# RhushabhVaghela/Custom-NVComp-with-ZSTD

Hardware: AMD Instinct MI355X
Metric: compress GB/s + ratio, 1 GB @ level 3, 64 KB chunks; libzstd round-trip OK (higher is better)
Workload: dtype u8; 1 GPU; C3: 16384 x 64 KiB chunks (1.00 GiB), level 3, independent frames; chunk_bytes=65536, chunks_total=16384, chunks_rank0=16384, level=3, parallelism=dp1 (contiguous chunk shards, RCCL all-gather of sizes inside the step), gathered_frame_bytes=388747049

## Files before the change

custom-nvcomp-with-zstd_amd/csrc/zh_lz.hip:

```cpp
#include "zh_common.h"
#include "zh_hash.h"
#include "zh_litpack.h"

#include <algorithm>
#include <vector>

#if defined(ZH_STAMPS) || defined(ZH_INS_CHECK)
__device__ u32 g_fixups;
extern "C" __global__ void zh_read_fixups(u32 *out) { *out = g_fixups; g_fixups = 0; }
extern "C" u32 zh_fixups_host() {
  u32 *d = nullptr, h = 0;
  if (hipMalloc(&d, 4) != hipSuccess) return ~0u;
  hipLaunchKernelGGL(zh_read_fixups, dim3(1), dim3(1), 0, 0, d);
  (void)hipMemcpy(&h, d, 4, hipMemcpyDeviceToHost);
  (void)hipFree(d);
  return h;
}
#endif
#ifdef ZH_TIMELINE
__device__ unsigned long long g_tl[16 * 8];
extern "C" __global__ void zh_read_timeline(unsigned long long *out) {
  for (u32 i = threadIdx.x; i < 16 * 8; i += blockDim.x) { out[i] = g_tl[i]; g_tl[i] = 0; }
}
extern "C" int zh_timeline_host(unsigned long long *out128) {
// ... 293 lines not shown
__device__ __forceinline__ u32 lookahead(const u32 *in32, const u16 *T, u32 we, u32 lim, u32 lane) {
  u32 cwe = 0;
  if (lane < 2 && we + lane < lim) {
    u32 lo, hi;
    ld64u(in32, we + lane, lo, hi);
    cwe = T[hash_of<LONG>(lo, hi)];
  }
  __asm__ volatile("" ::: "memory");
  return cwe;
}
struct NoCheck {
  __device__ bool operator()(bool) const { return true; }
};

template <bool LONG>
__device__ __forceinline__ void insert_span(const u32 *in32, u16 *T, u32 s, u32 e, u32 lane) {
  constexpr u32 JUNK = LONG ? HL_SIZE : HS_SIZE;
  for (u32 r = s; r < e; r += 64) {
    u32 const p = r + lane;
    bool const v = p < e;
    u32 lo, hi;
    ld64u(in32, v ? p : s, lo, hi);
    u32 const h = v ? hash_of<LONG>(lo, hi) : JUNK;
    T[h] = (u16)(p + 1);
    for (;;) {
      bool const lost = v && (u32)T[h] < p + 1;
      if (!__ballot(lost)) break;
      if (lost) T[h] = (u16)(p + 1);
    }
  }
  __asm__ volatile("" ::: "memory");
}

__device__ __forceinline__ bool skip_window(const u32 *misc, u32 k, u32 kskip0) {
  return k >= kskip0 && (u32)__builtin_amdgcn_readfirstlane(__atomic_load_n(&misc[MISC_NM + ((k - 3) & 3)], __ATOMIC_RELAXED)) == 0;
}
__device__ __forceinline__ bool skip_window_eff(const u32 *misc, u32 k, u32 kskip0) {
#ifdef ZH_NO_RESUME
  return skip_window(misc, k, kskip0);
#endif
  return skip_window(misc, k, kskip0) && (u32)__builtin_amdgcn_readfirstlane(__atomic_load_n(&misc[MISC_RESF + (k & 1)], __ATOMIC_RELAXED)) == 0;
}
template <bool LONG, bool TWO>
__device__ __forceinline__ bool resume_exchange(u32 *misc, u32 j, bool hit, u32 lane) {
  if constexpr (TWO) {
    u32 *const x = &misc[MISC_XCH + 2 * (j & 1)];
    if (lane == 0) __atomic_store_n(&x[LONG ? 1 : 0], ((j + 1) << 1) | (hit ? 1u : 0u), __ATOMIC_RELAXED);
    u32 v;
    for (;;) {
      v = (u32)__builtin_amdgcn_readfirstlane(__atomic_load_n(&x[LONG ? 0 : 1], __ATOMIC_RELAXED));
      if ((v >> 1) == j + 1) break;
      __builtin_amdgcn_s_sleep(1);
    }
    hit = hit || (v & 1u);
  }
  if (lane == 0) __atomic_store_n(&misc[MISC_RESF + (j & 1)], hit ? 1u : 0u, __ATOMIC_RELAXED);
  return hit;
}

__device__ __forceinline__ bool probe_dead(const u32 *misc, u32 k, u32 kprobe) {
  if (ZH_PROBE_WINDOWS == 1 || k != kprobe) return false;
  u32 m = 0;
#pragma unroll
  for (u32 j = 1; j <= ZH_PROBE_WINDOWS; j++) m |= __atomic_load_n(&misc[MISC_NM + ((k - 1 - j) & 3)], __ATOMIC_RELAXED);
  return (u32)__builtin_amdgcn_readfirstlane(m) == 0;
}
static_assert(ZH_PROBE_WINDOWS >= 1 && ZH_PROBE_WINDOWS <= 3, "probe windows fit the match-count ring");
constexpr u32 span_top_mask(u64 tab) {
  u32 m = 0, hi = 0;
  for (u32 w = 1; w + 1 < INS_TID / 64; w++) {
    hi += (u32)((tab >> (2 * w)) & 3u);
    m |= 1u << hi;
  }
  return m;
}
__device__ __forceinline__ bool span_top_dec(const u32 *ci, u32 wn, bool skip, u32 L, bool act) {
  constexpr u32 TOPS_FULL = span_top_mask(ROUND_TAB), TOPS_SKIP = ((1u << (2 * ZH_SKIP_TILES)) - 1u) & ~1u;
  u32 const hi = L + 1, i = 64 * hi - 1;
  bool const top = act && L < NROUND && (((skip ? TOPS_SKIP : TOPS_FULL) >> hi) & 1u) && i < wn;
  u32 const inf = top ? ci[cidx(i)] : 0u, inf1 = top ? ci[cidx(i + 1)] : 0u;
  return top && (inf & 255u) && (inf1 & 255u) <= (inf & 255u);
}
__device__ __forceinline__ bool probe_dead_tm(u32 k, u32 kprobe, u32 e0, bool lazy = false, u32 wnp = 0) {
  if (ZH_PROBE_WINDOWS != 1 || k + 1 != kprobe) return false;
  u8 *const smem = k1_lds();
  u32 lane;
  __asm__ volatile("v_mbcnt_lo_u32_b32 %0, -1, 0\n\tv_mbcnt_hi_u32_b32 %0, -1, %0" : "=v"(lane));
  const u64 *const tmP = (const u64 *)(smem + OFF_HM) + ((k & 1u) ^ 1u) * NROUND;
  u32 const r = lane & (NROUND - 1);
  u64 m = tmP[r];
  if (ZH_ONE_BARRIER && lazy) {
    const u32 *const ciP = (const u32 *)(smem + OFF_CI) + ((k & 1u) ^ 1u) * CI_WORDS;
    m |= span_top_dec(ciP, wnp, false, r, lane < NROUND) ? 1ull << 63 : 0ull;
  }
  u32 const lo = 64 * r;
  u64 const keep = e0 <= lo ? ~0ull : e0 >= lo + 64 ? 0ull : ~0ull << (e0 - lo);
  return __ballot(lane < NROUND && (m & keep) != 0) == 0;
}

template <bool LONG, u32 NT>
__device__ __forceinline__ void dump_window(u8 *ci8, u32 lane_, const u32 (&creg)[NCR], u32 cwe) {
  u32 lane;
  __asm__ volatile("v_mov_b32 %0, %1" : "=v"(lane) : "v"(lane_));
#pragma unroll
  for (u32 t = 0; t < NT; t++) {
#pragma unroll
    for (u32 k = 0; k < TPL; k++) {
      u32 const i = t * ZH_TILE + 64 * k + lane, j = t * TPL + k;
      u16 const v = (u16)(creg[j / 2] >> (16 * (j & 1)));
      *(u16 *)(ci8 + 4 * cidx(i) + (LONG ? 0 : 2)) = v;
    }
  }
  if (lane < 2) *(u16 *)(ci8 + 4 * cidx(ZH_WINDOW + lane) + (LONG ? 0 : 2)) = (u16)cwe;
}

__device__ __forceinline__ u32 bperm(u32 v, u32 src) { return (u32)__builtin_amdgcn_ds_bpermute((int)(src << 2), (int)v); }
__device__ __forceinline__ u32 ctz64(u64 v) { return (u32)__builtin_ctzll(v); }
__device__ __forceinline__ u32 bit_range32(u32 a, u32 b) {
  u32 const hi = b >= 32 ? ~0u : (1u << b) - 1u;
  return hi & ~((1u << a) - 1u);
}

template <u32 MODE>
__device__ __forceinline__ bool take_rule(u32 inf, u32 inf1) {
  if (MODE == 2) return true;
  return (inf1 & 255u) <= (inf & 255u);
}
template <u32 MODE>
constexpr bool two_tables() { return MODE == 0; }

__device__ __forceinline__ u32 ld4_before(const u32 *in32, u32 a) {
  u32 const t = a >= 4 ? a - 4 : 0u, w = t >> 2, sh = t & 3;
  u32 const v = __builtin_amdgcn_alignbyte(in32[w + 1], in32[w], sh);
  return a >= 4 ? v : v << (8 * (4 - a));
}
constexpr u32 MAX_RW = 3;
__device__ __forceinline__ u32 rounds_of(u32 w) {
#ifdef ZH_RTAB
  return (u32)(((unsigned long long)(ZH_RTAB) >> (2 * w)) & 3u);
#else
  return (u32)((ROUND_TAB >> (2 * w)) & 3u);
#endif
}

__device__ __forceinline__ void xq_flush(const u32 *in32, u32 *ci, const u16 *xq, u32 k, u32 wsb, u32 lane) {
  bool const act = lane < k;
  u32 const e = act ? xq[lane] : 0u;
  u32 const i = e & 0x1FFFu, sh = (e >> 15) * 16u;
  u32 const c = (ci[cidx(i)] >> sh) & 0xFFFFu;
  u32 const x = ext8(in32, act ? wsb + i : 0u, act && c ? c - 1u : 0u, act);
  if (act) ((u8 *)ci)[4 * cidx(i) + (sh >> 3)] = (u8)x;
}

enum : u32 { LF_FL = 1u << 8, LF_FS = 1u << 9, LF_XL = 1u << 10, LF_XS = 1u << 11, LF_SL = 1u << 12 };

template <u32 MODE>
__device__ __forceinline__ void span_lengths(const u32 *in32, u32 *ci, u64 *tm, u16 *xq, u32 r_lo, u32 r_hi, u32 wsb, u32 we, u32 n, u32 lim,
                                             u32 lane, bool top, u32 la1) {
  constexpr bool TWO = two_tables<MODE>();
  u32 cwr[MAX_RW], flg[MAX_RW];
  u32 olo[MAX_RW], ohi[MAX_RW], Lw[MAX_RW][3], Sw[MAX_RW][3];
  auto loadA = [&](u32 k) {
    u32 const r = r_hi - 1 - min(k, r_hi - 1 - r_lo), i = 64 * r + lane, p = wsb + i;
    u32 const cw = ci[cidx(i)];
    cwr[k] = cw;
    ld64u(in32, p, olo[k], ohi[k]);
    u32 const aL = ((cw - 1u) & 0xFFFFu) >> 2, aS = ((cw >> 16) + 0xFFFFu) >> 2 & 0x3FFFu;
#pragma unroll
    for (u32 t = 0; t < 3; t++) {
      if constexpr (TWO) Lw[k][t] = in32[aL + t];
      Sw[k][t] = in32[aS + t];
    }
  };
  u32 ccL = 0, ccS = 0;
  u32 nq = 0;
#pragma unroll
  for (u32 k = 0; k < MAX_RW; k++) {
    flg[k] = 0;
    if (r_lo + k >= r_hi) { cwr[k] = 0; continue; }
    loadA(k);
    u32 const r = r_hi - 1 - k, i = 64 * r + lane;
    u32 const cw = cwr[k];
    u32 const cL = TWO ? cw & 0xFFFFu : 0u, cS = cw >> 16;
    auto pref = [&](u32 c, const u32 (&w)[3]) {
      u32 const sh = (c - 1u) & 3u;
      u32 const x = olo[k] ^ __builtin_amdgcn_alignbyte(w[1], w[0], sh), y = ohi[k] ^ __builtin_amdgcn_alignbyte(w[2], w[1], sh);
      return min(ffbl_raw(x), min(ffbl_raw(y), 32u) + 32u) >> 3;
    };
    u32 const pL = TWO ? pref(cL, Lw[k]) : 0u, pS = pref(cS, Sw[k]);
    vpad<ZH_PAD_A>(pS);
    u32 cLn = wave_shl1(cL), cSn = wave_shl1(cS);
    cLn = lane == 63 ? ccL : cLn;
    cSn = lane == 63 ? ccS : cSn;
    bool const fL = pL == 8 && cLn == cL + 1u, fS = pS == 8 && cSn == cS + 1u;
    bool const xL = pL == 8 && !fL;
    bool const sL = cS == cL && xL && pS == 8 && !fS;
    bool const xS = pS == 8 && !fS && !sL;
    flg[k] = pL | (pS << 4) | (fL ? LF_FL : 0u) | (fS ? LF_FS : 0u) | (xL ? LF_XL : 0u) | (xS ? LF_XS : 0u) | (sL ? LF_SL : 0u);
    ccL = lane_value(cL, 0);
    ccS = lane_value(cS, 0);
    u64 const bL = TWO ? __ballot(xL) : 0ull, bS = __ballot(xS);
    u32 const rL = __builtin_amdgcn_mbcnt_hi((u32)(bL >> 32), __builtin_amdgcn_mbcnt_lo((u32)bL, 0u));
    u32 const rS = __builtin_amdgcn_mbcnt_hi((u32)(bS >> 32), __builtin_amdgcn_mbcnt_lo((u32)bS, 0u));
    u32 const nL = (u32)__popcll(bL);
    xq[xL ? nq + rL : XQ_CAP - 1] = (u16)i;
    xq[xS ? nq + nL + rS : XQ_CAP - 1] = (u16)(i | 0x8000u);
    nq = (u32)__builtin_amdgcn_readfirstlane(nq + nL + (u32)__popcll(bS));
    while (nq >= 64) {
      nq -= 64;
      xq_flush(in32, ci, xq + nq, 64, wsb, lane);
    }
  }
  if (nq) xq_flush(in32, ci, xq, nq, wsb, lane);
  u32 lLr[MAX_RW], lSr[MAX_RW], runs[MAX_RW];
  auto c1 = [&](u32 k) {
    u32 const r = r_hi - 1 - min(k, r_hi - 1 - r_lo), i = 64 * r + lane;
    u32 const f = flg[k];
    u32 const ce = ci[cidx(i)];
    u32 const pL = f & 15u, pS = (f >> 4) & 15u;
    u32 const eL = (f & LF_XL) ? (ce & 255u) : pL;
    u32 const eS = (f & LF_XS) ? ((ce >> 16) & 255u) : ((f & LF_SL) ? eL : pS);
    u64 const RS = __ballot(!(f & LF_FS)) >> lane;
    u32 const qS = RS ? ctz64(RS) : 64u - lane;
    u32 const vS = bperm(eS, min(lane + qS, 63u));
    lSr[k] = RS ? min((u32)ZH_MAX_MATCH, qS + vS) : qS;
    runs[k] = RS ? 0u : 2u;
    if constexpr (TWO) {
      u64 const RL = __ballot(!(f & LF_FL)) >> lane;
      u32 const qL = RL ? ctz64(RL) : 64u - lane;
      u32 const vL = bperm(eL, min(lane + qL, 63u));
      lLr[k] = RL ? min((u32)ZH_MAX_MATCH, qL + vL) : qL;
      runs[k] |= RL ? 0u : 1u;
    } else {
      lLr[k] = 0;
    }
  };
#pragma unroll
  for (u32 k = 0; k < MAX_RW; k++) c1(k);
  u32 clL = 0, clS = 0;
  u32 cv1 = la1;
#pragma unroll
  for (u32 k = 0; k < MAX_RW; k++) {
    if (r_lo + k >= r_hi) continue;
    u32 const r = r_hi - 1 - k, i = 64 * r + lane, p = wsb + i;
    u32 const cw = cwr[k];
    u32 const cL = TWO ? cw & 0xFFFFu : 0u, cS = cw >> 16;
    u32 const lL = (runs[k] & 1u) ? min((u32)ZH_MAX_MATCH, lLr[k] + clL) : lLr[k];
    u32 const lS = (runs[k] & 2u) ? min((u32)ZH_MAX_MATCH, lSr[k] + clS) : lSr[k];
    vpad<ZH_PAD_C>(lS);
    clL = lane_value(lL, 0);
    clS = lane_value(lS, 0);
    u32 const capj = min((u32)ZH_MAX_MATCH, n - min(p, n));
    u32 const rL = min(lL, capj), rS = min(lS, capj);
    u32 const mL = (cL && rL >= ZH_MIN_MATCH_LONG) ? rL : 0u;
    u32 const mS = (cS && rS >= ZH_MIN_MATCH_SHORT) ? rS : 0u;
    bool const useL = mL && mL >= mS;
    u32 const ml = useL ? mL : mS, cm = useL ? cL : cS;
    u32 const v = ml ? ((p - (cm - 1u)) << 8) | ml : 0u;
    u32 v1 = wave_shl1(v);
    v1 = lane == 63 ? cv1 : v1;
    cv1 = lane_value(v, 0);
    bool const unk = MODE != 2 && k == 0 && !top && lane == 63;
    bool const tk = v != 0 && !unk && take_rule<MODE>(v, v1);
    ci[cidx(i)] = v;
    u64 const tb = __ballot(tk);
    if (lane == 0) tm[r] = tb;
  }
}

constexpr u32 L1_S = ZH_L1_STRIDE;
constexpr u32 NROUND1 = NROUND / L1_S;
static_assert(L1_S == 1 || L1_S == 2 || L1_S == 4, "level-1 stride");
__device__ __forceinline__ u64 spread_bits(u64 v, u32 s) {
  if (s == 2) {
    v = (v | (v << 16)) & 0x0000FFFF0000FFFFull;
    v = (v | (v << 8)) & 0x00FF00FF00FF00FFull;
    v = (v | (v << 4)) & 0x0F0F0F0F0F0F0F0Full;
    v = (v | (v << 2)) & 0x3333333333333333ull;
    v = (v | (v << 1)) & 0x5555555555555555ull;
  } else if (s == 4) {
    v = (v | (v << 24)) & 0x000000FF000000FFull;
    v = (v | (v << 12)) & 0x000F000F000F000Full;
    v = (v | (v << 6)) & 0x0303030303030303ull;
    v = (v | (v << 3)) & 0x1111111111111111ull;
  }
  return v;
}
__device__ __forceinline__ void span_lengths_l1(const u32 *in32, u32 *ci, u64 *tm, u16 *xq, u32 r_lo, u32 r_hi, u32 wsb, u32 n, u32 lane) {
  constexpr u32 S = L1_S;
  u32 cwr[MAX_RW], flg[MAX_RW], olo[MAX_RW], ohi[MAX_RW], Sw[MAX_RW][3];
  auto loadA = [&](u32 k) {
    u32 const r = r_hi - 1 - min(k, r_hi - 1 - r_lo), i = 64 * S * r + S * lane, p = wsb + i;
    u32 const cw = ci[cidx(i)];
    cwr[k] = cw;
    ld64u(in32, p, olo[k], ohi[k]);
    u32 const aS = ((cw >> 16) + 0xFFFFu) >> 2 & 0x3FFFu;
#pragma unroll
    for (u32 t = 0; t < 3; t++) Sw[k][t] = in32[aS + t];
  };
  u32 ccS = 0, nq = 0;
#pragma unroll
  for (u32 k = 0; k < MAX_RW; k++) {
    flg[k] = 0;
    if (r_lo + k >= r_hi) { cwr[k] = 0; continue; }
    loadA(k);
    u32 const r = r_hi - 1 - k, i = 64 * S * r + S * lane;
    u32 const cS = cwr[k] >> 16;
    u32 const sh = (cS - 1u) & 3u;
    u32 const x = olo[k] ^ __builtin_amdgcn_alignbyte(Sw[k][1], Sw[k][0], sh), y = ohi[k] ^ __builtin_amdgcn_alignbyte(Sw[k][2], Sw[k][1], sh);
    u32 const pS = min(ffbl_raw(x), min(ffbl_raw(y), 32u) + 32u) >> 3;
    u32 cSn = wave_shl1(cS);
    cSn = lane == 63 ? ccS : cSn;
    bool const fS = pS == 8 && cSn == cS + S;
    bool const xS = pS == 8 && !fS;
    flg[k] = (pS << 4) | (fS ? LF_FS : 0u) | (xS ? LF_XS : 0u);
    ccS = lane_value(cS, 0);
    u64 const bS = __ballot(xS);
    u32 const rS = __builtin_amdgcn_mbcnt_hi((u32)(bS >> 32), __builtin_amdgcn_mbcnt_lo((u32)bS, 0u));
    xq[xS ? nq + rS : XQ_CAP - 1] = (u16)(i | 0x8000u);
    nq = (u32)__builtin_amdgcn_readfirstlane(nq + (u32)__popcll(bS));
    while (nq >= 64) {
      nq -= 64;
      xq_flush(in32, ci, xq + nq, 64, wsb, lane);
    }
  }
  if (nq) xq_flush(in32, ci, xq, nq, wsb, lane);
  u32 lSr[MAX_RW], runs[MAX_RW];
#pragma unroll
  for (u32 k = 0; k < MAX_RW; k++) {
    u32 const r = r_hi - 1 - min(k, r_hi - 1 - r_lo), i = 64 * S * r + S * lane;
    u32 const f = flg[k];
    u32 const ce = ci[cidx(i)];
    u32 const eS = (f & LF_XS) ? ((ce >> 16) & 255u) : ((f >> 4) & 15u);
    u64 const RS = __ballot(!(f & LF_FS)) >> lane;
    u32 const qS = RS ? ctz64(RS) : 64u - lane;
    u32 const vS = bperm(eS, min(lane + qS, 63u));
    lSr[k] = RS ? min((u32)ZH_MAX_MATCH, S * qS + vS) : S * qS;
    runs[k] = RS ? 0u : 2u;
  }
  u32 clS = 0;
#pragma unroll
  for (u32 k = 0; k < MAX_RW; k++) {
    if (r_lo + k >= r_hi) continue;
    u32 const r = r_hi - 1 - k, i = 64 * S * r + S * lane, p = wsb + i;
    u32 const cS = cwr[k] >> 16;
    u32 const lS = (runs[k] & 2u) ? min((u32)ZH_MAX_MATCH, lSr[k] + clS) : lSr[k];
    clS = lane_value(lS, 0);
    u32 const capj = min((u32)ZH_MAX_MATCH, n - min(p, n));
    u32 const rS = min(lS, capj);
    u32 const mS = (cS && rS >= ZH_MIN_MATCH_SHORT) ? rS : 0u;
    u32 const v = mS ? ((p - (cS - 1u)) << 8) | mS : 0u;
    ci[cidx(i)] = v;
    u64 const tb = __ballot(v != 0);
    if (lane == 0) {
#pragma unroll
      for (u32 s = 0; s < S; s++) tm[S * r + s] = S == 1 ? tb : spread_bits((tb >> (64 / S * s)) & ((1ull << (64 / S)) - 1ull), S);
    }
  }
}
constexpr u64 ROUND_TAB1 = 0x5556664ull;
static_assert(L1_S != 2 || (((ROUND_TAB1 >> 2) & 3) + ((ROUND_TAB1 >> 4) & 3) + ((ROUND_TAB1 >> 6) & 3) + ((ROUND_TAB1 >> 8) & 3) +
                            ((ROUND_TAB1 >> 10) & 3) + ((ROUND_TAB1 >> 12) & 3) + ((ROUND_TAB1 >> 14) & 3) + ((ROUND_TAB1 >> 16) & 3) +
                            ((ROUND_TAB1 >> 18) & 3) + ((ROUND_TAB1 >> 20) & 3) + ((ROUND_TAB1 >> 22) & 3) + ((ROUND_TAB1 >> 24) & 3) +
                            ((ROUND_TAB1 >> 26) & 3)) == NROUND1, "level-1 round table covers the window");
template <u32 MODE>
__device__ __forceinline__ u32 rounds_of_mode(u32 w) {
  if constexpr (MODE == 2 && L1_S == 2) {
#ifdef ZH_RTAB1
    return (u32)(((unsigned long long)(ZH_RTAB1) >> (2 * w)) & 3u);
#else
    return (u32)((ROUND_TAB1 >> (2 * w)) & 3u);
#endif
  } else if constexpr (MODE == 2 && L1_S == 4) {
    return w >= 1 && w <= 8 ? 1u : 0u;
  } else {
    return rounds_of(w);
  }
}

template <u32 MODE>
__device__ __forceinline__ u32 info_one(const u32 *in32, u32 p, u32 cw, u32 n, u32 lim, bool act) {
  bool const hv = act && p < lim;
  u32 const cL = (hv && two_tables<MODE>()) ? (cw & 0xFFFFu) : 0u, cS = hv ? (cw >> 16) : 0u;
  u32 lo, hi;
  ld64u(in32, hv ? p : 0u, lo, hi);
  u32 const tL = prefix8(in32, cL ? cL - 1u : 0u, lo, hi), tS = prefix8(in32, cS ? cS - 1u : 0u, lo, hi);
  u32 const pL = cL ? tL : 0u, pS = cS ? tS : 0u;
  u32 const e1 = ext8(in32, pL == 8 ? p : 0u, pL == 8 ? cL - 1u : 0u, pL == 8);
  u32 const e2 = ext8(in32, pS == 8 ? p : 0u, pS == 8 ? cS - 1u : 0u, pS == 8);
  u32 const lL = pL == 8 ? e1 : pL, lS = pS == 8 ? e2 : pS;
  u32 const capj = min((u32)ZH_MAX_MATCH, n - min(p, n));
  u32 const rL = min(lL, capj), rS = min(lS, capj);
  u32 const mL = (cL && rL >= ZH_MIN_MATCH_LONG) ? rL : 0u;
  u32 const mS = (cS && rS >= ZH_MIN_MATCH_SHORT) ? rS : 0u;
  bool const useL = mL && mL >= mS;
  u32 const ml = useL ? mL : mS, cm = useL ? cL : cS;
  return ml ? ((p - (cm - 1u)) << 8) | ml : 0u;
}

__device__ __forceinline__ u32 catch_up(const u32 *in32, u32 P, u32 off, u32 lo, bool act) {
  u32 maxe = (act && P > lo && P > off) ? min(P - lo, P - off) : 0u;
  u32 e = 0;
  while (__ballot(e < maxe)) {
    if (e < maxe) {
      u32 const a = P - e, x = ld4_before(in32, a) ^ ld4_before(in32, a - off);
      u32 const m = x ? (u32)__builtin_clz(x) >> 3 : 4u;
      e += min(m, maxe - e);
      maxe = m < 4 ? e : maxe;
    }
  }
  return e;
}

template <bool REWALK, typename LenQ>
__device__ __forceinline__ void seg_walk(LenQ &&lenq, u32 tmk, u32 S, u32 SE, u32 p, bool act0, u32 &LM, u32 &MM, u32 &ex) {
  u32 const old = (REWALK && act0) ? (LM | MM) : 0u;
  vpad<ZH_PAD_W>(p);
  u32 nl = 0, nm = 0;
// ... 402 lines not shown
      in[i] = c;
      same &= i < pre || c == first;
    }
  } else {
    u8 const first = src[0];
    for (u32 i = tid; i < n; i += K1_THREADS) { u8 c = src[i]; in[i] = c; same &= c == first; }
  }
  if (tid < 16) in[n + tid] = 0;
  bool const use_dt = ws.dtab && (d.flags & ZH_F_DICT) && (d.flags & ZH_F_FIRST) && pre >= 2 * ZH_DTAB_MARGIN && d.n >= 16 &&
                      ws.dtab_P >= pre;
  bool const par_hist = !use_dt && pre >= 2 * ZH_TILE && d.n >= 16;
  u32 const pmin = (use_dt || par_hist) ? pre & ~(ZH_TILE - 1) : 0u;
  u32 const wstart = (use_dt || par_hist) ? (pre & ~(ZH_WINDOW - 1)) : 0u;
  u32 const span_s = use_dt ? pre - ZH_DTAB_MARGIN : 0u, span_e = use_dt ? pmin : 0u;
#ifdef ZH_NO_SKIP
  u32 const kskip0 = 1u << 20;
#else
  u32 const kskip0 = pre / ZH_WINDOW + 3 - wstart / ZH_WINDOW;
#endif
  u32 const lim = n > ZH_HASH_READ ? n - ZH_HASH_READ : 0;
  u32 const a0 = pre / ZH_WINDOW, nwl = (lim + ZH_WINDOW - 1) / ZH_WINDOW;
  u32 const e0p = pre - a0 * ZH_WINDOW;
  u32 const kprobe0 = a0 + ZH_PROBE_WINDOWS + 1 <= nwl && e0p <= ZH_PROBE_MAX_E0 ? a0 + ZH_PROBE_WINDOWS + 1 - wstart / ZH_WINDOW : ~0u;
  u32 next_b = 0;
  if (use_dt) {
    u32 const delta = ws.dtab_P - pre;
    const u32 *dt32 = (const u32 *)ws.dtab;
    auto clip = [&](u32 e) { return e > delta ? e - delta : 0u; };
    for (u32 i = tid; i < (HL_SIZE + HS_SIZE) / 2; i += K1_THREADS) {
      u32 const w = dt32[i];
      u32 const v = clip(w & 0xFFFFu) | (clip(w >> 16) << 16);
      u32 const j = i < HL_SIZE / 2 ? i : i + T_PAD / 2;
      ((u32 *)TL)[j] = v;
    }
    if (tid < T_PAD) ((u16 *)TL)[tid < T_PAD / 2 ? HL_SIZE + tid : HL_SIZE + T_PAD + HS_SIZE + (tid - T_PAD / 2)] = 0;
  } else {
    for (u32 i = tid; i < (HL_SIZE + HS_SIZE + 2 * T_PAD) / 2; i += K1_THREADS) ((u32 *)TL)[i] = 0;
  }
  if (tid == 0) {
    misc[MISC_ARR] = 0;
#pragma unroll
    for (u32 i = 0; i < 4; i++) misc[MISC_XCH + i] = 0;
  }
  if (!redo) {
    bool const rle = !block_any(!same, &misc[MISC_ANY], tid) && d.n >= 2;
    next_b = *s_take;
    prefetch_block(blocks, next_b, nblocks, tid, pf);
    if (rle) {
      if (tid == 0) {
        u32 one;
        __asm__ volatile("v_mov_b32 %0, 1" : "=v"(one));
        meta[0] = one - 1u; meta[1] = one - 1u; meta[2] = one;
      }
      return next_b;
    }
  } else {
    next_b = *s_take;
    k1_barrier();
  }
  if (par_hist) {
    for (u32 round = 0;; round++) {
      bool ch = false;
      for (u32 p = tid; p < pmin; p += K1_THREADS) {
        u32 lo, hi;
        ld64u(in32, p, lo, hi);
        u32 const hl = hash_of<true>(lo, hi), hs = hash_of<false>(lo, hi);
        u16 const v = (u16)(p + 1);
        if (round == 0) {
          TL[hl] = v;
          TS[hs] = v;
        } else {
          if (TL[hl] < v) { TL[hl] = v; ch = true; }
          if (TS[hs] < v) { TS[hs] = v; ch = true; }
        }
      }
      if (round == 0) k1_barrier();
      else if (!block_any(ch, &misc[MISC_ANY], tid)) break;
    }
  }

  ZH_STAMP(st_stage);
  u32 const kprobe = redo ? ~0u : kprobe0;
  bool dead = false;
  if (tid >= INS_TID) {
    __builtin_amdgcn_s_setprio(2);
    bool const lw = tid < INS_TID + 64;
    LitJob<two_tables<MODE>()> lj{in32, (u32 *)(smem + OFF_SEGM), (u32 *)(smem + OFF_LB), ws.lits(b), wstart, n, pre,
              two_tables<MODE>() && !lw ? LIT_ROUNDS / 2 : 0u, two_tables<MODE>() ? LIT_ROUNDS / 2 : (lw ? LIT_ROUNDS : 0u), 0u};
    if (tid >= INS_TID + 64)
      dead = inserter_loop<false, two_tables<MODE>()>(in32, TS, ci8, misc, n, lim, lane, ws.dbg(b), wstart, pmin, span_s, span_e, kskip0, kprobe, e0p, lj,
                                                      MODE != 2);
    else if (two_tables<MODE>())
      dead = inserter_loop<true, true>(in32, TL, ci8, misc, n, lim, lane, ws.dbg(b), wstart, pmin, span_s, span_e, kskip0, kprobe, e0p, lj, MODE != 2);
    else
      dead = idle_inserter_loop(misc, n, wstart, kprobe, e0p, lj, lane, MODE != 2);
    __builtin_amdgcn_s_setprio(0);
    if (!dead) return next_b;
  } else {
  u64 *const seq_out = ws.seq(b);
  u32 nseq_tot = 0, nlit_tot = 0, e_in = pre;
  u32 const tid_ = tid;
  u32 const wave = tid >> 6;
  u32 r_lo = 0;
  for (u32 w = 0; w < wave; w++) r_lo += rounds_of_mode<MODE>(w);
  u32 const r_hi = r_lo + rounds_of_mode<MODE>(wave);
  u32 *const ci0 = ci;
  u32 *const sgm = (u32 *)(smem + OFF_SEGM);
  u32 *const lbx = (u32 *)(smem + OFF_LB);
  u16 *const xq = (u16 *)(smem + OFF_XQ) + XQ_CAP * wave;
  u32 const nwin = (n - wstart + ZH_WINDOW - 1) / ZH_WINDOW;
  u64 *const mlist = (u64 *)(smem + OFF_ML);
  u32 nwalk_tot = 0;
  TL_DECL;
  u32 m3 = 0;
  bool skp_prev = false;
  for (u32 k = 0; k < nwin + STEPS_EXTRA; k++, m3 = m3 + 1 == LM_BUFS ? 0u : m3 + 1) {
    if (probe_dead(misc, k, kprobe)) {
      dead = true;
      break;
    }
    u32 const wsb = wstart + k * ZH_WINDOW;
    u32 const we = min(wsb + ZH_WINDOW, n);
    u32 const kb = k & 1u;
    bool const have = k < nwin && we > pre;
    u32 const wsp = wsb - ZH_WINDOW, wep = min(wsp + ZH_WINDOW, n);
    bool const prev = k >= 1 && k <= nwin && wep > pre;
    u32 const wsq = wsb - 2 * ZH_WINDOW;
    bool const prev2 = k >= 2 && k - 2 < nwin && min(wsq + ZH_WINDOW, n) > pre;
    u32 tid;
    __asm__ volatile("v_mov_b32 %0, %1" : "=v"(tid) : "v"(tid_));
    u32 const lane = tid & 63;
    u32 *const ciK = ci0 + kb * CI_WORDS, *const ciP = ci0 + (kb ^ 1u) * CI_WORDS;
    u64 *const tmK = hm + kb * NROUND, *const tmP = hm + (kb ^ 1u) * NROUND;
    static_assert(LM_BUFS == 3 && LB_BUFS == 2, "literal buffer rotation");
    u32 *const lmP = sgm + segm(m3 == 0 ? 2u : m3 - 1u);
    u32 *const lmQ = sgm + segm(m3 == 0 ? 1u : m3 == 1 ? 2u : 0u);
    u32 *const lbxq = lbx + kb * LB_WORDS;
    u64 *const mlP = mlist + (kb ^ 1u) * ML_CAP, *const mlQ = mlist + kb * ML_CAP;
    k1_barrier();
    TL_MARK(0);
    TL_STEP();
    if (probe_dead_tm(k, kprobe, e0p, MODE != 2, wep - wsp)) {
      dead = true;
      break;
    }
    ZH_STAMP(st_A);
    constexpr u32 RS = 2 * ZH_SKIP_TILES;
    static_assert(RS < NWW && (RS & 1) == 0, "miss-skip rounds");
    bool const skipk = have && skip_window_eff(misc, k, kskip0);
    if (skipk && wave != 0) {
      if constexpr (MODE == 2) {
        if (wave <= RS / L1_S) span_lengths_l1(in32, ciK, tmK, xq, wave - 1, wave, wsb, n, lane);
      } else {
        if (wave <= RS) span_lengths<MODE>(in32, ciK, tmK, xq, wave - 1, wave, wsb, we, n, lim, lane, wave == RS, 0u);
      }
      for (u32 r = RS + wave - 1; r < NROUND; r += NWW - 1) {
        ciK[cidx(64 * r + lane)] = 0;
        if (lane == 0) tmK[r] = 0;
      }
      ZH_STAMP(st_B);
    } else if (MODE == 2 && have && wave != 0) {
      if (r_lo < r_hi) span_lengths_l1(in32, ciK, tmK, xq, r_lo, r_hi, wsb, n, lane);
      ZH_STAMP(st_B);
    } else if (have && wave != 0) {
      u32 la1 = 0;
      if (wave == NWW - 1) {
        u32 const p = we + lane;
        u32 const cw = ciK[cidx(ZH_WINDOW + (lane & 1))];
        u32 const li = info_one<MODE>(in32, p, cw, n, lim, MODE != 2 && lane == 0 && p < n);
        if (lane < 2) ciK[cidx(ZH_WINDOW + lane)] = li;
        la1 = lane_value(li, 0);
      }
      span_lengths<MODE>(in32, ciK, tmK, xq, r_lo, r_hi, wsb, we, n, lim, lane, wave == NWW - 1, la1);
      ZH_STAMP(st_B);
    }
    TL_MARK(1);
    if (wave == 0 && prev) {
      u32 const wn = wep - wsp;
      u32 const S = SEGP * lane, SE = min(S + SEGP, wn);
      u32 tmk = (u32)(tmP[lane >> 1] >> (32 * (lane & 1)));
      if constexpr (ZH_ONE_BARRIER && MODE != 2) {
        bool const dt = span_top_dec(ciP, wn, skp_prev, lane, lane < NROUND);
        u32 const d = bperm(dt ? 1u : 0u, (lane - 1u) >> 1);
        tmk |= ((lane & 1u) && d) ? 1u << 31 : 0u;
      }
      u32 const e0 = e_in - wsp;
      u32 entry = lane == 0 ? e0 : max(S, e0), ex = entry;
      u32 LM = 0, MM = 0;
      auto lenq = [&](u32 q) { return ciP[cidx(q)] & 255u; };
      seg_walk<false>(lenq, tmk, S, SE, entry, true, LM, MM, ex);
      for (;;) {
#if ZH_K1_PMAX
        u32 const pe = wave_shr1(wave_scan_max_incl(ex));
#else
        u32 const pe = wave_shr1(ex);
#endif
        u32 const ne = lane == 0 ? e0 : max(pe, e0);
        bool const ch = ne != entry;
#ifdef ZH_STAMPS
        st_rounds++;
#endif
        if (!__ballot(ch)) break;
        seg_walk<true>(lenq, tmk, S, SE, ne, ch, LM, MM, ex);
        entry = ne;
      }
      e_in = wsp + lane_value(ex, 63);
      ZH_STAMP(st_J1);
      u32 const ns = (u32)__popc(MM);
      u32 const is = wave_scan_incl(ns);
      u32 const nm = lane_value(is, 63);
      lmP[lane] = LM;
      u32 const nwl = lane_value(wave_scan_incl((u32)__popc(LM)), 63);
      u32 mm = MM, q = is - ns;
      while (__ballot(mm != 0)) {
        if (mm) {
          mlP[q++] = S + (u32)__builtin_ctz(mm);
          mm &= mm - 1u;
        }
      }
      ZH_STAMP(st_J2);
      u32 covered = 0, pend = e0;
      for (u32 j0 = 0; j0 < nm; j0 += 64) {
        u32 const j = j0 + lane;
        bool const v = j < nm;
        u32 const ms = v ? (u32)mlP[j] : 0u, inf = ciP[cidx(ms)];
        u32 const len = v ? inf & 255u : 0u, off = (inf >> 8) & 0xFFFFu;
        u32 const incl = wave_scan_incl(len);
        u32 const cum = nwalk_tot + (ms - e0) - (covered + incl - len);
        u32 lo = wave_shr1(ms + len);
        if (lane == 0) lo = pend;
        pend = lane_value(ms + len, min(63u, nm - 1u - j0));
        covered += lane_value(incl, 63);
        if (v) mlP[j] = (u64)ms | ((u64)lo << ML_LO) | ((u64)len << ML_LEN) | ((u64)off << ML_OFF) | ((u64)cum << ML_CUM);
      }
      nwalk_tot += nwl;
      if (lane == 0) { misc[MISC_WNM + (kb ^ 1u)] = nm; misc[MISC_NM + ((k - 1) & 3)] = nm; }
      ZH_STAMP(st_J);
    }
    if (ZH_ONE_BARRIER && wave == 0 && lane == 0) __atomic_store_n(&misc[MISC_PF], k + 1, __ATOMIC_RELAXED);
    if (wave == REC_WAVE && prev2) {
      u32 const nm = (u32)__builtin_amdgcn_readfirstlane(misc[MISC_WNM + kb]);
      for (u32 j0 = 0; j0 < nm; j0 += 64) {
        u32 const j = j0 + lane;
        bool const v = j < nm;
        u64 const en = v ? mlQ[j] : 0ull;
        u32 const ms = (u32)en & 0x7FFu, lo = (u32)(en >> ML_LO) & 0x7FFu, len = (u32)(en >> ML_LEN) & 0x7Fu;
        u32 const off = (u32)(en >> ML_OFF) & 0xFFFFu, cum = (u32)(en >> ML_CUM);
        u32 const e = catch_up(in32, wsq + ms, off, wsq + lo, v);
        if (v) seq_out[nseq_tot + j] = (u64)cum | ((u64)len << 17) | ((u64)e << 24) | ((u64)off << 36);
        if (e) {
          for (u32 g = (ms - e) / SEGP; g <= (ms - 1) / SEGP; g++) {
            u32 const a = max(ms - e, SEGP * g) - SEGP * g, bnd = min(ms - SEGP * g, SEGP);
            atomicAnd(&lmQ[g], ~bit_range32(a, bnd));
          }
        }
      }
      u32 const lc = (u32)__popc(lmQ[lane]), lincl = wave_scan_incl(lc);
      lbxq[lane] = lincl - lc;
      if (lane == 63) lbxq[NSEG] = lincl;
      if (ZH_ONE_BARRIER) {
        nlit_tot += lane_value(lincl, 63);
        nseq_tot += nm;
      }
    }
    TL_MARK(2);
    if (!ZH_ONE_BARRIER) {
      if (lane == 0) atomicAdd(&misc[MISC_ARR], 1u);
      k1_barrier();
    }
    TL_MARK(3);
    ZH_STAMP(st_X);
    if (!ZH_ONE_BARRIER && MODE != 2 && have && wave != 0 && wave < (skipk ? RS : NWW - 1)) {
      u32 const hi = skipk ? wave : r_hi;
      u32 const i = 64 * hi - 1;
      if (lane == 0) {
        u32 const inf = ciK[cidx(i)], inf1 = ciK[cidx(i + 1)];
        if (i < we - wsb && (inf & 255u) && take_rule<MODE>(inf, inf1)) atomicOr((u32 *)&tmK[i >> 6] + ((i >> 5) & 1u), 1u << (i & 31));
      }
    }
    if (ZH_ONE_BARRIER) {
    } else if (prev2) {
      nlit_tot += (u32)__builtin_amdgcn_readfirstlane(lbxq[NSEG]);
      nseq_tot += __builtin_amdgcn_readfirstlane(misc[MISC_WNM + kb]);
    }
    ZH_STAMP(st_E);
    TL_MARK(4);
    skp_prev = skipk;
  }
  TL_FLUSH(wave, lane);
  if (!dead) {
    if (tid_ == (ZH_ONE_BARRIER ? 64u * REC_WAVE : 0u)) { meta[0] = nseq_tot; meta[1] = nlit_tot; meta[2] = 0; }
#ifdef ZH_STAMPS
    if (tid == 0) {
      u32 *dbg = ws.dbg(b);
      dbg[23] = (u32)rt0; dbg[24] = (u32)__builtin_amdgcn_s_memrealtime();
      dbg[25] = __builtin_amdgcn_s_getreg((31 << 11) | 4);
      dbg[26] = __builtin_amdgcn_s_getreg((31 << 11) | 20);
      dbg[27] = (u32)(__builtin_amdgcn_s_memtime() - mt0);
      dbg[40] = st_Bmax; dbg[41] = st_Imax; dbg[55] = st_J1; dbg[56] = st_J2; dbg[57] = st_J3;
      dbg[0] = st_stage; dbg[1] = st_A; dbg[2] = st_B; dbg[3] = st_J; dbg[4] = st_E; dbg[5] = st_rounds; dbg[20] = st_E2; dbg[21] = st_X; dbg[22] = st_E1;
    }
    if ((tid & 63) == 0 && tid < INS_TID) {
      u32 const w = tid >> 6;
#ifdef ZH_EXP_PWAIT
      ws.dbg(b)[w < 12 ? 28 + w : 53 + (w - 12)] = st_A;
#else
      ws.dbg(b)[w < 12 ? 28 + w : 53 + (w - 12)] = st_B;
// ... 170 lines not shown
```

custom-nvcomp-with-zstd_amd/cuda_zstd/__init__.py:

```python
from __future__ import annotations

import ctypes
import os
from typing import List, Sequence

_HERE = os.path.dirname(os.path.abspath(__file__))
LIB_PATH = os.environ.get("CUDA_ZSTD_HIP_LIB") or os.path.join(os.path.dirname(_HERE), "libcuda_zstd_hip.so")

OK, INVALID, OOM, DEVICE_ERROR, CORRUPT, TOO_SMALL, CHECKSUM, COMPRESSION = 0, 2, 3, 4, 6, 7, 10, 12

_lib = None


class ZstdError(RuntimeError):
    def __init__(self, code: int, what: str = ""):
        self.code = code
        super().__init__(f"{what}: {error_string(code)} (code {code})")


def lib() -> ctypes.CDLL:
    global _lib
    if _lib is None:
        if not os.path.exists(LIB_PATH):
            raise ImportError(f"{LIB_PATH} not found: build it with __graft_entry__.build() (make -C custom-nvcomp-with-zstd_amd)")
        L = ctypes.CDLL(LIB_PATH)
        vp, sz, i = ctypes.c_void_p, ctypes.c_size_t, ctypes.c_int
        psz, pvp, pi = ctypes.POINTER(sz), ctypes.POINTER(vp), ctypes.POINTER(i)
        sig = {
            "cuda_zstd_create_manager": (vp, [i]),
            "cuda_zstd_destroy_manager": (None, [vp]),
            "cuda_zstd_compress": (i, [vp, vp, sz, vp, psz, vp, sz, vp]),
            "cuda_zstd_decompress": (i, [vp, vp, sz, vp, psz, vp, sz, vp]),
            "cuda_zstd_get_compress_workspace_size": (sz, [vp, sz]),
            "cuda_zstd_get_decompress_workspace_size": (sz, [vp, sz]),
            "cuda_zstd_get_max_compressed_size": (sz, [vp, sz]),
            "cuda_zstd_get_batch_compress_workspace_size": (sz, [vp, psz, sz]),
            "cuda_zstd_compress_batch": (i, [vp, pvp, psz, sz, pvp, psz, pi, vp, sz, vp]),
            "cuda_zstd_get_error_string": (ctypes.c_char_p, [i]),
            "cuda_zstd_is_error": (i, [i]),
            "cuda_zstd_train_dictionary": (vp, [pvp, psz, sz, sz]),
            "cuda_zstd_load_dictionary": (vp, [vp, sz]),
            "cuda_zstd_destroy_dictionary": (None, [vp]),
            "cuda_zstd_set_dictionary": (i, [vp, vp]),
            "cuda_zstd_clear_dictionary": (i, [vp]),
            "cuda_zstd_get_dictionary_content": (sz, [vp, vp, sz]),
            "cuda_zstd_get_dictionary_layout": (i, [vp, ctypes.POINTER(ctypes.c_uint), psz]),
            "nvcomp_zstd_batch_create_v5": (vp, [i, ctypes.c_uint, i]),
            "nvcomp_zstd_batch_destroy_v5": (None, [vp]),
            "nvcomp_zstd_batch_get_compress_temp_size_v5": (sz, [vp, psz, sz]),
            "nvcomp_zstd_batch_get_max_compressed_chunk_size_v5": (sz, [vp, sz]),
            "nvcomp_zstd_batch_compress_async_v5": (i, [vp, vp, vp, sz, vp, vp, vp, sz, vp]),
            "nvcomp_zstd_batched_compress_get_temp_size_v5": (sz, [sz, sz]),
            "nvcomp_zstd_batch_get_batched_temp_size_v5": (sz, [vp, sz, sz]),
            "nvcomp_zstd_batch_set_dictionary_v5": (i, [vp, vp]),
            "nvcomp_zstd_batched_compress_async_v5": (i, [vp, vp, vp, sz, sz, vp, vp, vp, vp, sz, vp]),
            "cuda_zstd_get_batch_decompress_workspace_size": (sz, [vp, psz, sz]),
            "cuda_zstd_decompress_batch": (i, [vp, pvp, psz, sz, pvp, psz, pi, vp, sz, vp]),
            "nvcomp_zstd_batch_get_decompress_temp_size_v5": (sz, [vp, psz, sz]),
            "nvcomp_zstd_batch_decompress_async_v5": (i, [vp, vp, vp, sz, vp, vp, vp, sz, vp]),
            "nvcomp_zstd_batched_decompress_get_temp_size_v5": (sz, [sz, sz]),
            "nvcomp_zstd_batched_decompress_async_v5": (i, [vp, vp, vp, vp, sz, sz, vp, vp, vp, vp, sz, vp]),
            "cuda_zstd_write_metadata_frame": (i, [vp, sz, i, psz, vp]),
            "cuda_zstd_stream_create": (vp, [i]),
            "cuda_zstd_stream_destroy": (None, [vp]),
            "cuda_zstd_stream_compress_chunk": (i, [vp, vp, sz, vp, psz, i, i, vp]),
            "cuda_zstd_stream_decompress_chunk": (i, [vp, vp, sz, vp, psz, pi, vp]),
            "cuda_zstd_stream_reset": (i, [vp]),
            "cuda_zstd_hybrid_create": (vp, [vp]),
            "cuda_zstd_hybrid_create_default": (vp, []),
            "cuda_zstd_hybrid_destroy": (None, [vp]),
            "cuda_zstd_hybrid_compress": (i, [vp, vp, sz, vp, psz, ctypes.c_uint, ctypes.c_uint, vp, vp]),
            "cuda_zstd_hybrid_decompress": (i, [vp, vp, sz, vp, psz, ctypes.c_uint, ctypes.c_uint, vp, vp]),
            "cuda_zstd_hybrid_max_compressed_size": (sz, [vp, sz]),
            "cuda_zstd_hybrid_query_routing": (ctypes.c_uint, [vp, sz, ctypes.c_uint, ctypes.c_uint, i]),
            "cuda_zstd_extract_metadata": (i, [vp, sz, ctypes.POINTER(ctypes.c_uint), ctypes.POINTER(ctypes.c_ulonglong), ctypes.POINTER(ctypes.c_uint), pi]),
            "cuda_zstd_hip_version": (ctypes.c_char_p, []),
            "cuda_zstd_hip_profile_enable": (None, [i]),
            "cuda_zstd_hip_profile_collect": (i, [ctypes.POINTER(ctypes.c_double)]),
            "cuda_zstd_hip_kernel_lds_bytes": (ctypes.c_uint, [i]),
            "cuda_zstd_seekable_max_size": (sz, [sz, sz, i]),
            "cuda_zstd_seekable_pack_get_temp_size": (sz, [sz]),
            "cuda_zstd_seekable_pack_async": (i, [vp, vp, vp, vp, vp, sz, sz, i, vp, sz, vp, vp, vp, sz, vp]),
            "cuda_zstd_seekable_info": (i, [vp, sz, psz, ctypes.POINTER(ctypes.c_ulonglong), ctypes.POINTER(ctypes.c_uint), pi]),
            "cuda_zstd_seekable_read_get_temp_size": (sz, [sz, sz]),
            "cuda_zstd_seekable_read_get_temp_size_jobs": (sz, [sz, sz, sz]),
            "cuda_zstd_seekable_read": (i, [vp, vp, sz, ctypes.c_ulonglong, sz, vp, psz, i, vp, sz, vp]),
        }
        for name, (res, args) in sig.items():
            f = getattr(L, name)
            f.restype = res
            f.argtypes = args
        _lib = L
    return _lib


def error_string(code: int) -> str:
    return lib().cuda_zstd_get_error_string(code).decode()


def _torch():
    import torch

    if not torch.cuda.is_available():
        raise RuntimeError("cuda_zstd: no GPU visible (the gfx950 path has no CPU fallback)")
    return torch


def _stream_ptr(stream) -> int:
    torch = _torch()
    s = stream if stream is not None else torch.cuda.current_stream()
    return s.cuda_stream


def max_compressed_size(n: int) -> int:
    nb = max(1, (n + 128 * 1024 - 1) // (128 * 1024))
    return n + n // 255 + nb * 3 + 512


MIN_LEVEL, MAX_LEVEL, DEFAULT_LEVEL = 1, 22, 3
__version__ = "0.2.0"


def _is_host(x) -> bool:
    return isinstance(x, (bytes, bytearray, memoryview)) or type(x).__module__.startswith("numpy")


def _to_device(x):
    torch = _torch()
    import numpy as np

    a = np.frombuffer(bytes(x), np.uint8) if isinstance(x, (bytes, bytearray, memoryview)) else np.ascontiguousarray(x).view(np.uint8).reshape(-1)
    if a.size == 0:
        return torch.empty(0, dtype=torch.uint8, device="cuda")
    return torch.from_numpy(a.copy()).cuda()


def _host_bytes(t) -> bytes:
    return t.cpu().numpy().tobytes() if t.numel() else b""


def _frame_size(frame) -> int:
    try:
        return extract_metadata(frame)["uncompressed_size"] or frame.numel() * 16
    except ZstdError:
        return max(frame.numel() * 16, 1024)


class Manager:

    def __init__(self, level: int = 3):
        self.level = level
        self._h = lib().cuda_zstd_create_manager(level)
        if not self._h:
            raise ZstdError(INVALID, "cuda_zstd_create_manager")
        self._ws = None

    def close(self):
        if self._h:
            lib().cuda_zstd_destroy_manager(self._h)
            self._h = None

    def __del__(self):
        try:
            self.close()
        except Exception:
            pass

    def __enter__(self):
        return self

    def __exit__(self, *exc):
        self.close()
        return False

    def __repr__(self):
        return f"<cuda_zstd.Manager level={self.level}>"

# ... 572 lines not shown
```

Before: 85.55 GB/s.

## Rework span_lengths match-run scan with wave masks, packed subtraction and byte permutes

Rewrites the per-round match-length pass in span_lengths. Per-lane flag words are replaced by wave-wide 64-bit masks. Candidate neighbour comparison uses a single DPP shift of the packed candidate word and a packed 16-bit subtract. The per-lane length extraction becomes a single v_perm with precomputed selectors, and run carry-in is computed from the first-run position instead of per-lane ballots and selects. The round bounds are made wave-uniform, and the skip path instantiates a one-round specialisation. The aim is fewer VALU ops, ballots and VGPRs in this hot loop, at the risk of subtle length/carry semantics changes (clL-6, clS-7 offsets) that must still match the previous output.

```diff
diff --git a/custom-nvcomp-with-zstd_amd/csrc/zh_lz.hip b/custom-nvcomp-with-zstd_amd/csrc/zh_lz.hip
--- a/custom-nvcomp-with-zstd_amd/csrc/zh_lz.hip
+++ b/custom-nvcomp-with-zstd_amd/csrc/zh_lz.hip
@@ -469,101 +469,115 @@
   if (act) ((u8 *)ci)[4 * cidx(i) + (sh >> 3)] = (u8)x;
 }
 
-enum : u32 { LF_FL = 1u << 8, LF_FS = 1u << 9, LF_XL = 1u << 10, LF_XS = 1u << 11, LF_SL = 1u << 12 };
-
-template <u32 MODE>
-__device__ __forceinline__ void span_lengths(const u32 *in32, u32 *ci, u64 *tm, u16 *xq, u32 r_lo, u32 r_hi, u32 wsb, u32 we, u32 n, u32 lim,
+enum : u32 { LF_FS = 1u << 9, LF_XS = 1u << 11 };
+
+__device__ __forceinline__ u64 mask_of(bool b) { return __builtin_amdgcn_ballot_w64(b); }
+__device__ __forceinline__ bool lane_of(u64 m) { return __builtin_amdgcn_inverse_ballot_w64(m); }
+typedef unsigned short u16x2 __attribute__((ext_vector_type(2)));
+__device__ __forceinline__ u32 pk_sub16(u32 a, u32 b) {
+  return __builtin_bit_cast(u32, (u16x2)(__builtin_bit_cast(u16x2, a) - __builtin_bit_cast(u16x2, b)));
+}
+
+template <u32 MODE, u32 NR = MAX_RW>
+__device__ __forceinline__ void span_lengths(const u32 *in32, u32 *ci, u64 *tm, u16 *xq, u32 r_lo_, u32 r_hi_, u32 wsb, u32 we, u32 n, u32 lim,
                                              u32 lane, bool top, u32 la1) {
   constexpr bool TWO = two_tables<MODE>();
-  u32 cwr[MAX_RW], flg[MAX_RW];
-  u32 olo[MAX_RW], ohi[MAX_RW], Lw[MAX_RW][3], Sw[MAX_RW][3];
+  u32 const r_lo = (u32)__builtin_amdgcn_readfirstlane(r_lo_), r_hi = r_lo + (u32)__builtin_amdgcn_readfirstlane(r_hi_ - r_lo_);
+  auto has_round = [&](u32 k) {
+    u32 h = r_hi;
+    __asm__ volatile("" : "+s"(h));
+    return r_lo + k < h;
+  };
+  static_assert(ZH_MIN_MATCH_LONG == 8 && ZH_MAX_MATCH <= 255, "pass A: the long side keeps only `8 bytes equal`");
+  u32 cwr[NR], cm1[NR], pp[NR], sel[NR];
+  u64 mFL[NR], mFS[NR];
+  u32 olo[NR], ohi[NR], Lw[NR][3], Sw[NR][3];
   auto loadA = [&](u32 k) {
     u32 const r = r_hi - 1 - min(k, r_hi - 1 - r_lo), i = 64 * r + lane, p = wsb + i;
     u32 const cw = ci[cidx(i)];
     cwr[k] = cw;
     ld64u(in32, p, olo[k], ohi[k]);
-    u32 const aL = ((cw - 1u) & 0xFFFFu) >> 2, aS = ((cw >> 16) + 0xFFFFu) >> 2 & 0x3FFFu;
-#pragma unroll
-    for (u32 t = 0; t < 3; t++) {
-      if constexpr (TWO) Lw[k][t] = in32[aL + t];
-      Sw[k][t] = in32[aS + t];
+    u32 const t = pk_sub16(cw, 0x00010001u);
+    cm1[k] = t;
+    const u8 *const in8 = (const u8 *)in32;
+    const u32 *const wL = (const u32 *)(in8 + (t & 0xFFFCu)), *const wS = (const u32 *)(in8 + ((t >> 16) & 0xFFFCu));
+#pragma unroll
+    for (u32 j = 0; j < 3; j++) {
+      if constexpr (TWO) Lw[k][j] = wL[j];
+      Sw[k][j] = wS[j];
     }
   };
-  u32 ccL = 0, ccS = 0;
+  u32 ccw = 0;
   u32 nq = 0;
 #pragma unroll
-  for (u32 k = 0; k < MAX_RW; k++) {
-    flg[k] = 0;
-    if (r_lo + k >= r_hi) { cwr[k] = 0; continue; }
+  for (u32 k = 0; k < NR; k++) {
+    mFL[k] = mFS[k] = 0;
+    pp[k] = sel[k] = 0;
+    if (!has_round(k)) continue;
     loadA(k);
     u32 const r = r_hi - 1 - k, i = 64 * r + lane;
-    u32 const cw = cwr[k];
-    u32 const cL = TWO ? cw & 0xFFFFu : 0u, cS = cw >> 16;
-    auto pref = [&](u32 c, const u32 (&w)[3]) {
-      u32 const sh = (c - 1u) & 3u;
-      u32 const x = olo[k] ^ __builtin_amdgcn_alignbyte(w[1], w[0], sh), y = ohi[k] ^ __builtin_amdgcn_alignbyte(w[2], w[1], sh);
-      return min(ffbl_raw(x), min(ffbl_raw(y), 32u) + 32u) >> 3;
+    u32 const cw = cwr[k], t = cm1[k];
+    auto diff = [&](u32 sh, const u32 (&w)[3], u32 &x, u32 &y) {
+      x = olo[k] ^ __builtin_amdgcn_alignbyte(w[1], w[0], sh & 3u);
+      y = ohi[k] ^ __builtin_amdgcn_alignbyte(w[2], w[1], sh & 3u);
     };
-    u32 const pL = TWO ? pref(cL, Lw[k]) : 0u, pS = pref(cS, Sw[k]);
+    u32 xs, ys, xl = 1, yl = 0;
+    diff(t >> 16, Sw[k], xs, ys);
+    if constexpr (TWO) diff(t, Lw[k], xl, yl);
+    u32 const pS = min(ffbl_raw(xs), min(ffbl_raw(ys), 32u) + 32u) >> 3;
     vpad<ZH_PAD_A>(pS);
-    u32 cLn = wave_shl1(cL), cSn = wave_shl1(cS);
-    cLn = lane == 63 ? ccL : cLn;
-    cSn = lane == 63 ? ccS : cSn;
-    bool const fL = pL == 8 && cLn == cL + 1u, fS = pS == 8 && cSn == cS + 1u;
-    bool const xL = pL == 8 && !fL;
-    bool const sL = cS == cL && xL && pS == 8 && !fS;
-    bool const xS = pS == 8 && !fS && !sL;
-    flg[k] = pL | (pS << 4) | (fL ? LF_FL : 0u) | (fS ? LF_FS : 0u) | (xL ? LF_XL : 0u) | (xS ? LF_XS : 0u) | (sL ? LF_SL : 0u);
-    ccL = lane_value(cL, 0);
-    ccS = lane_value(cS, 0);
-    u64 const bL = TWO ? __ballot(xL) : 0ull, bS = __ballot(xS);
+    u32 const cwn = (u32)__builtin_amdgcn_update_dpp((int)ccw, (int)cw, 0x130, 0xf, 0xf, false);
+    u32 const d = pk_sub16(cwn, cw);
+    u64 const m8L = TWO ? mask_of(xl == 0) & mask_of(yl == 0) : 0ull, m8S = mask_of(pS == 8);
+    u64 const mnL = TWO ? mask_of((d & 0xFFFFu) == 1u) : 0ull, mnS = mask_of((d >> 16) == 1u);
+    u64 const bL = m8L & ~mnL, eS8 = m8S & ~mnS;
+    u64 const mSL = TWO ? mask_of((cw >> 16) == (cw & 0xFFFFu)) & bL & eS8 : 0ull;
+    u64 const bS = eS8 & ~mSL;
+    mFL[k] = m8L & mnL;
+    mFS[k] = m8S & mnS;
+    bool const xL = lane_of(bL), xS = lane_of(bS), sL = lane_of(mSL);
+    pp[k] = 7u | pS << 16;
+    sel[k] = (xL ? 0x0C020C04u : 0x0C020C00u) + (xS ? 0x40000u : sL ? 0x20000u : 0u);
+    ccw = lane_value(cw, 0);
     u32 const rL = __builtin_amdgcn_mbcnt_hi((u32)(bL >> 32), __builtin_amdgcn_mbcnt_lo((u32)bL, 0u));
     u32 const rS = __builtin_amdgcn_mbcnt_hi((u32)(bS >> 32), __builtin_amdgcn_mbcnt_lo((u32)bS, 0u));
-    u32 const nL = (u32)__popcll(bL);
+    u32 const nqL = nq + (u32)__popcll(bL);
     xq[xL ? nq + rL : XQ_CAP - 1] = (u16)i;
-    xq[xS ? nq + nL + rS : XQ_CAP - 1] = (u16)(i | 0x8000u);
-    nq = (u32)__builtin_amdgcn_readfirstlane(nq + nL + (u32)__popcll(bS));
+    xq[xS ? nqL + rS : XQ_CAP - 1] = (u16)(i | 0x8000u);
+    nq = nqL + (u32)__popcll(bS);
+#pragma nounroll
     while (nq >= 64) {
       nq -= 64;
       xq_flush(in32, ci, xq + nq, 64, wsb, lane);
     }
   }
   if (nq) xq_flush(in32, ci, xq, nq, wsb, lane);
-  u32 lLr[MAX_RW], lSr[MAX_RW], runs[MAX_RW];
+  u32 lLr[NR], lSr[NR];
   auto c1 = [&](u32 k) {
     u32 const r = r_hi - 1 - min(k, r_hi - 1 - r_lo), i = 64 * r + lane;
-    u32 const f = flg[k];
-    u32 const ce = ci[cidx(i)];
-    u32 const pL = f & 15u, pS = (f >> 4) & 15u;
-    u32 const eL = (f & LF_XL) ? (ce & 255u) : pL;
-    u32 const eS = (f & LF_XS) ? ((ce >> 16) & 255u) : ((f & LF_SL) ? eL : pS);
-    u64 const RS = __ballot(!(f & LF_FS)) >> lane;
-    u32 const qS = RS ? ctz64(RS) : 64u - lane;
-    u32 const vS = bperm(eS, min(lane + qS, 63u));
-    lSr[k] = RS ? min((u32)ZH_MAX_MATCH, qS + vS) : qS;
-    runs[k] = RS ? 0u : 2u;
+    u32 const e = __builtin_amdgcn_perm(ci[cidx(i)], pp[k], sel[k]);
+    u32 const qS = ctz64((~mFS[k] | 1ull << 63) >> lane);
+    lSr[k] = qS + (bperm(e, lane + qS) >> 16);
     if constexpr (TWO) {
-      u64 const RL = __ballot(!(f & LF_FL)) >> lane;
-      u32 const qL = RL ? ctz64(RL) : 64u - lane;
-      u32 const vL = bperm(eL, min(lane + qL, 63u));
-      lLr[k] = RL ? min((u32)ZH_MAX_MATCH, qL + vL) : qL;
-      runs[k] |= RL ? 0u : 1u;
+      u32 const qL = ctz64((~mFL[k] | 1ull << 63) >> lane);
+      lLr[k] = qL + (bperm(e, lane + qL) & 255u);
     } else {
       lLr[k] = 0;
     }
   };
 #pragma unroll
-  for (u32 k = 0; k < MAX_RW; k++) c1(k);
+  for (u32 k = 0; k < NR; k++) c1(k);
   u32 clL = 0, clS = 0;
   u32 cv1 = la1;
 #pragma unroll
-  for (u32 k = 0; k < MAX_RW; k++) {
-    if (r_lo + k >= r_hi) continue;
+  for (u32 k = 0; k < NR; k++) {
+    if (!has_round(k)) continue;
     u32 const r = r_hi - 1 - k, i = 64 * r + lane, p = wsb + i;
     u32 const cw = cwr[k];
     u32 const cL = TWO ? cw & 0xFFFFu : 0u, cS = cw >> 16;
-    u32 const lL = (runs[k] & 1u) ? min((u32)ZH_MAX_MATCH, lLr[k] + clL) : lLr[k];
-    u32 const lS = (runs[k] & 2u) ? min((u32)ZH_MAX_MATCH, lSr[k] + clS) : lSr[k];
+    auto first_run = [](u64 f) { return ~f ? 64u - (u32)__builtin_clzll(~f) : 0u; };
+    u32 const lL = min((u32)ZH_MAX_MATCH, lLr[k] + (lane >= first_run(mFL[k]) ? clL - 6u : 0u));
+    u32 const lS = min((u32)ZH_MAX_MATCH, lSr[k] + (lane >= first_run(mFS[k]) ? clS - 7u : 0u));
     vpad<ZH_PAD_C>(lS);
     clL = lane_value(lL, 0);
     clS = lane_value(lS, 0);
@@ -577,10 +591,9 @@
     u32 v1 = wave_shl1(v);
     v1 = lane == 63 ? cv1 : v1;
     cv1 = lane_value(v, 0);
-    bool const unk = MODE != 2 && k == 0 && !top && lane == 63;
-    bool const tk = v != 0 && !unk && take_rule<MODE>(v, v1);
+    u64 const unk = MODE != 2 && k == 0 && !top ? 1ull << 63 : 0ull;
     ci[cidx(i)] = v;
-    u64 const tb = __ballot(tk);
+    u64 const tb = mask_of(v != 0) & mask_of(take_rule<MODE>(v, v1)) & ~unk;
     if (lane == 0) tm[r] = tb;
   }
 }
@@ -1289,7 +1302,7 @@
       if constexpr (MODE == 2) {
         if (wave <= RS / L1_S) span_lengths_l1(in32, ciK, tmK, xq, wave - 1, wave, wsb, n, lane);
       } else {
-        if (wave <= RS) span_lengths<MODE>(in32, ciK, tmK, xq, wave - 1, wave, wsb, we, n, lim, lane, wave == RS, 0u);
+        if (wave <= RS) span_lengths<MODE, 1>(in32, ciK, tmK, xq, wave - 1, wave, wsb, we, n, lim, lane, wave == RS, 0u);
       }
       for (u32 r = RS + wave - 1; r < NROUND; r += NWW - 1) {
         ciK[cidx(64 * r + lane)] = 0;
diff --git a/custom-nvcomp-with-zstd_amd/cuda_zstd/__init__.py b/custom-nvcomp-with-zstd_amd/cuda_zstd/__init__.py
--- a/custom-nvcomp-with-zstd_amd/cuda_zstd/__init__.py
+++ b/custom-nvcomp-with-zstd_amd/cuda_zstd/__init__.py
@@ -23,6 +23,10 @@
     if _lib is None:
         if not os.path.exists(LIB_PATH):
             raise ImportError(f"{LIB_PATH} not found: build it with __graft_entry__.build() (make -C custom-nvcomp-with-zstd_amd)")
+        try:
+            import torch
+        except ImportError:
+            pass
         L = ctypes.CDLL(LIB_PATH)
         vp, sz, i = ctypes.c_void_p, ctypes.c_size_t, ctypes.c_int
         psz, pvp, pi = ctypes.POINTER(sz), ctypes.POINTER(vp), ctypes.POINTER(i)
```

Result: faster. 89.34 GB/s, median of 6 (+4.4%).
